# TDLdefA-QUN/Noise-Resilience-in-Discrete-Time-Crystal-Realizations-on-Quantum-Computers

Measured on AMD Instinct MI355X. Metric: Floquet-periods×instances/sec at L=20; RZZ-kernel HBM GB/s vs peak, higher is better.
Workload: dtype f64

## Files before the change

noise-resilience-in-discrete-time-crystal-realizations-on-quantum-computers_amd/csrc/dtc_lightcone.hip:

```cpp
#include <cstdlib>
#include <type_traits>

#include "dtc_device.h"
#include "dtc_kernels.h"

#ifndef DTC_LCW3_WPS
#if defined(DTC_LCW3_ADD) || defined(DTC_LCW3_MERGE)
#define DTC_LCW3_WPS 3
#else
#define DTC_LCW3_WPS 4
#endif
#endif
#ifndef DTC_LCW2_WPS
#define DTC_LCW2_WPS 4
#endif

namespace dtc {

static constexpr int kLcTilesPerGroup = 2;

template <int KIND, int TPB, bool SPLIT = false>
__device__ __forceinline__ void lc_body(const PassArgs& A) {
  static_assert(KIND == kKindRX || KIND == kKindRY, "light-cone pass: factored kicks");
  __shared__ double2 s_tile[SPLIT ? 1 : kTile];
  __shared__ double s_half[SPLIT ? kHalfSlots : 1];
  __shared__ double2 s_cone[kLcTab4];
  __shared__ double s_red[kThreads / 64][2];
  const int t = threadIdx.x;
  const int c = A.c, s = A.s;
  const int64_t n_tiles = (int64_t)1 << (A.L_eff - kTileBits);
  const int og = A.octet_bits;
  const int64_t b = og ? (((int64_t)blockIdx.y << 3) | (blockIdx.x & 7)) : (int64_t)blockIdx.y;
  const int64_t tile0 = (og ? (int64_t)(blockIdx.x >> 3) : (int64_t)blockIdx.x) * TPB;
  if (og && b >= A.batch) return;
  const int inst = (int)((A.batch_start + b) / A.n_traj);
  const RecScalar R(A.recs + b * kRecPerState);
  const int64_t mid_mask = ((int64_t)1 << A.tile_bits_mid) - 1;
  TileMap M;
  M.c = c;
  M.s = s;
  M.cmask = (1 << c) - 1;
  auto tbase_of = [&](int64_t tile) {
    return ((tile & mid_mask) << c) | ((tile >> A.tile_bits_mid) << (s + kTileBits - c));
  };
  M.tbase = tbase_of(tile0);
  constexpr int kConePerThread = (kLcTab4 + kThreads - 1) / kThreads;
  double2 cv[kConePerThread];
  const double2* ct = A.lc_diag + (int64_t)inst * kLcTab;
#pragma unroll
  for (int j = 0; j < kConePerThread; ++j) {
    const int i = t + j * kThreads;
    if (i < kLcTab4) cv[j] = ct[i];
  }
  const int64_t vofs = octet_spread(M.rel(ybase<2>(t)), og) << 4;
  const char* src = (const char*)(A.src + state_base(b, A.state_len, og));
  auto load_tile = [&](double2 (&dst)[kRegs], int64_t tb) {
#pragma unroll
    for (int r = 0; r < kRegs; ++r) {
      const char* a = src + (octet_spread(tb | M.rel(r << 8), og) << 4) + vofs;
      const d2v w = __builtin_nontemporal_load((const d2v*)a);
      dst[r] = make_double2(w.x, w.y);
    }
  };
  double2 v[kRegs];
  load_tile(v, M.tbase);
  __builtin_amdgcn_s_waitcnt(0x4F70);
  const double cs = A.diag_conj ? -1.0 : 1.0;
#pragma unroll
  for (int j = 0; j < kConePerThread; ++j) {
    const int i = t + j * kThreads;
    if (i < kLcTab4) s_cone[i] = make_double2(cv[j].x, cs * cv[j].y);
  }
  const double g2 = R.d(0, kLcG2);
  const long long packed = R.bits(kLcPacked);
  const int nl = A.lc_layers;
  const int jp = A.probe;

  auto kick = [&](double2 (&v)[kRegs], auto n_tag, auto l_tag) {
    constexpr int N = decltype(n_tag)::value;
    constexpr int l = decltype(l_tag)::value;
    constexpr int k0 = kLcSites * l + 4 * (N - 1);
    const int m = (int)((A.lc_mask >> k0) & 0xFull);
    if (m & 1) layer_f<KIND, 0, 0>(v, R.d(0, k0));
    if (m & 2) layer_f<KIND, 0, 1>(v, R.d(0, k0 + 1));
    if (m & 4) layer_f<KIND, 0, 2>(v, R.d(0, k0 + 2));
    if (m & 8) layer_f<KIND, 0, 3>(v, R.d(0, k0 + 3));
  };
  auto diag = [&](double2 (&v)[kRegs], auto lay_tag, int l) {
    constexpr int LAY = decltype(lay_tag)::value;
    const int rad = nl - 1 - l;
    const int lo = max(0, jp - rad), hi = min(A.L_real - 1, jp + rad);
    const int msk = (1 << (hi - lo + 1)) - 1;
    const int g0 = s + 4 * LAY - c;
    const int64_t m = (int64_t)((packed >> (8 * l)) & 0xFF) << s;
    const int base = (int)(((M.at(ybase<LAY>(t)) ^ m) >> lo) & msk);
    const double2* tab = s_cone + lc_tab_off(rad);
#pragma unroll
    for (int r = 0; r < kRegs; ++r) {
      const int off = (g0 >= lo ? (r << (g0 - lo)) : (r >> (lo - g0))) & msk;
      const int i = base ^ off;
      v[r] = cmul(v[r], tab[rad == 4 ? lc_pos4(i) : i]);
    }
  };
  using L1 = std::integral_constant<int, 1>;
  using L2 = std::integral_constant<int, 2>;
  auto lc_xch_impl = [&](double2 (&v)[kRegs], auto from_tag, auto to_tag) {
    constexpr int F = decltype(from_tag)::value, T = decltype(to_tag)::value;
    if constexpr (SPLIT) exchange_split<F, T>(v, s_half, t);
    else exchange<F, T>(v, s_tile, t);
  };
  auto process = [&](double2 (&v)[kRegs], int64_t tile) {
    M.tbase = tbase_of(tile);
    kick(v, L2{}, std::integral_constant<int, 0>{});
    lc_xch_impl(v, std::integral_constant<int, 2>{}, std::integral_constant<int, 1>{});
    kick(v, L1{}, std::integral_constant<int, 0>{});
    if (nl > 1) {
      diag(v, L1{}, 0);
      kick(v, L1{}, std::integral_constant<int, 1>{});
      lc_xch_impl(v, std::integral_constant<int, 1>{}, std::integral_constant<int, 2>{});
      kick(v, L2{}, std::integral_constant<int, 1>{});
    }
    if (nl > 2) {
      diag(v, L2{}, 1);
      kick(v, L2{}, std::integral_constant<int, 2>{});
      lc_xch_impl(v, std::integral_constant<int, 2>{}, std::integral_constant<int, 1>{});
      kick(v, L1{}, std::integral_constant<int, 2>{});
    }
    if (nl > 3) {
      diag(v, L1{}, 2);
      kick(v, L1{}, std::integral_constant<int, 3>{});
      lc_xch_impl(v, std::integral_constant<int, 1>{}, std::integral_constant<int, 2>{});
      kick(v, L2{}, std::integral_constant<int, 3>{});
    }
    if (nl > 4) {
      diag(v, L2{}, 3);
      kick(v, L2{}, std::integral_constant<int, 4>{});
      lc_xch_impl(v, std::integral_constant<int, 2>{}, std::integral_constant<int, 1>{});
      kick(v, L1{}, std::integral_constant<int, 4>{});
    }
    const int lay = (nl & 1) ? 1 : 2;
    double ptot = 0.0, pz = 0.0;
    {
      const int64_t x0 = lay == 1 ? M.at(ybase<1>(t)) : M.at(ybase<2>(t));
      const int tb = jp < c ? jp : ((jp >= s && jp < s + kTileBits - c) ? c + jp - s : -1);
      const int jr = tb - 4 * lay;
#pragma unroll
      for (int r = 0; r < kRegs; ++r) {
        const double p2 = fma(v[r].x, v[r].x, v[r].y * v[r].y);
        ptot += p2;
        pz += (jr >= 0 && jr < 4 && ((r >> jr) & 1)) ? -p2 : p2;
      }
      if (!(jr >= 0 && jr < 4)) pz = ((x0 >> jp) & 1) ? -ptot : ptot;
      if ((packed >> (32 + jp - s)) & 1) pz = -pz;
    }
    const int wave = t >> 6, lane = t & 63;
    const double tot = wave_sum(ptot) * g2;
    const double z = wave_sum(pz) * g2;
    if (lane == 0) {
      s_red[wave][0] = tot;
      s_red[wave][1] = z;
    }
    __syncthreads();
    if (t < 2) {
      double acc = 0.0;
// ... 358 lines not shown
#pragma unroll
    for (int p = 4; p < 12; ++p) xl |= (uint32_t)((t >> (p - 4)) & 1) << gpos(lay_site(kL0, p));
    const int64_t vofs = octet_spread((int64_t)xl, og) << 4;
    const char* src = (const char*)(A.src + state_base(b, A.state_len, og));
    const int64_t sp0 = octet_spread((int64_t)tbase, og) << 4;
    int64_t spq[4];
#pragma unroll
    for (int q = 0; q < 4; ++q) spq[q] = octet_spread((int64_t)1 << gpos(lay_site(kL0, q)), og) << 4;
#pragma unroll
    for (int r = 0; r < kRegs; ++r) {
      int64_t o = sp0;
#pragma unroll
      for (int q = 0; q < 4; ++q)
        if ((r >> q) & 1) o += spq[q];
      const d2v w = *(const d2v*)(src + o + vofs);
      v[r] = make_double2(w.x, w.y);
    }
  }
  const double2* ct = A.lc_diag + (int64_t)inst * kLcTab;
  auto tab_of = [](int e) {
    return e >= tab_off(kT1) ? kT1 : e >= tab_off(kT2) ? kT2 : e >= tab_off(kT3) ? kT3
         : e >= tab_off(kT4b) ? kT4b : e >= tab_off(kT4a) ? kT4a : e >= tab_off(kT5b) ? kT5b : kT5a;
  };
  auto tab_start = [](int k) {
    return k == kT5a ? tab_off(kT5a) : k == kT5b ? tab_off(kT5b) : k == kT4a ? tab_off(kT4a)
         : k == kT4b ? tab_off(kT4b) : k == kT3 ? tab_off(kT3) : k == kT2 ? tab_off(kT2) : tab_off(kT1);
  };
  auto src_of = [](int k) {
    return k == kT5a ? tab_src(kT5a) : k == kT5b ? tab_src(kT5b) : k == kT4a ? tab_src(kT4a)
         : k == kT4b ? tab_src(kT4b) : k == kT3 ? tab_src(kT3) : k == kT2 ? tab_src(kT2) : tab_src(kT1);
  };
  const int e1 = t + kThreads;
  const int k0 = tab_of(t), k1 = tab_of(e1);
  const int i0 = t - tab_start(k0), i1 = e1 - tab_start(k1);
  const double2 tv0 = ct[src_of(k0) + (k0 == kT5a ? lc_pos5a(i0) : i0)];
  double2 tv1 = make_double2(0.0, 0.0);
  if (e1 < kTabEntries) tv1 = ct[src_of(k1) + i1];
  kick(C0{}, C0{}, LCW2_SITE(m2));
  kick(C1{}, C0{}, LCW2_SITE(m1));
  kick(C2{}, C0{}, LCW2_SITE(z0));
  kick(C3{}, C0{}, LCW2_SITE(p1));
  {
    const double cs = A.diag_conj ? -1.0 : 1.0;
    const uint64_t m0 = (uint64_t)R.bits(kLcwMask + 0), m1 = (uint64_t)R.bits(kLcwMask + 1);
    const uint64_t m2 = (uint64_t)R.bits(kLcwMask + 2), m3 = (uint64_t)R.bits(kLcwMask + 3);
    const uint64_t m4 = (uint64_t)R.bits(kLcwMask + 4);
    auto stage = [&](int k, int i, double2 tv) {
      const int l = tab_layer(k);
      const uint64_t m = l == 0 ? m0 : l == 1 ? m1 : l == 2 ? m2 : l == 3 ? m3 : m4;
      const int lo = k == kT5a ? -5 : k == kT4a ? -4 : k == kT3 ? -3 : k == kT2 ? -2 : k == kT1 ? -1 : 0;
      const int nb = k == kT3 ? 7 : (k == kT5a || k == kT5b) ? 6 : k == kT1 ? 3 : 5;
      const int x = i ^ (int)((m >> (j + lo)) & ((1u << nb) - 1u));
      const int pos = k == kT5a ? (((x & 7) << 3) | (x >> 3))
                    : k == kT3 ? (((x & 15) << 2) | ((x >> 4) & 3) | (x & 64)) : x;
      s_tab[tab_start(k) + pos] = make_double2(tv.x, cs * tv.y);
    };
    stage(k0, i0, tv0);
    if (e1 < kTabEntries) stage(k1, i1, tv1);
  }

  xch(std::integral_constant<int, kL0>{}, std::integral_constant<int, kL1>{});
  kick(C0{}, C0{}, LCW2_SITE(m5));
  kick(C1{}, C0{}, LCW2_SITE(m4));
  kick(C2{}, C0{}, LCW2_SITE(m3));
  {
    int ba = tab_base<kL1, kT5a>(t, bit_p5), bb = tab_base<kL1, kT5b>(t, bit_p5);
    asm volatile("" : "+v"(ba), "+v"(bb));
    const double2* ta = s_tab + tab_off(kT5a) + ba;
    const double2* tb = s_tab + tab_off(kT5b) + bb;
#pragma unroll
    for (int r = 0; r < 8; ++r) {
      const double2 f = ta[tab_reg<kL1, kT5a>(r)];
      v[r] = cmul(v[r], f);
      v[r + 8] = cmul(v[r + 8], f);
    }
    const double2 f0 = tb[0], f1 = tb[tab_reg<kL1, kT5b>(8)];
#pragma unroll
    for (int r = 0; r < 8; ++r) {
      v[r] = cmul(v[r], f0);
      v[r + 8] = cmul(v[r + 8], f1);
    }
  }
  kick(C1{}, C1{}, LCW2_SITE(m4));
  kick(C2{}, C1{}, LCW2_SITE(m3));
  kick(C3{}, C1{}, LCW2_SITE(p4));
  xch(std::integral_constant<int, kL1>{}, std::integral_constant<int, kL2s>{});
  kick(C0{}, C1{}, LCW2_SITE(m2));
  kick(C1{}, C1{}, LCW2_SITE(m1));
  kick(C2{}, C1{}, LCW2_SITE(z0));
  kick(C3{}, C1{}, LCW2_SITE(p1));
  swap_reg_lane<0, 16>(v);
  swap_reg_lane<1, 32>(v);
  kick(C0{}, C1{}, LCW2_SITE(p2));
  kick(C1{}, C1{}, LCW2_SITE(p3));
  {
    int ba = tab_base<kL2e, kT4a>(t, bit_p5), bb = tab_base<kL2e, kT4b>(t, bit_p5);
    asm volatile("" : "+v"(ba), "+v"(bb));
    const double2* ta = s_tab + tab_off(kT4a) + ba;
    const double2* tb = s_tab + tab_off(kT4b) + bb;
    const double2 a0 = ta[0], a1 = ta[tab_reg<kL2e, kT4a>(4)];
#pragma unroll
    for (int r = 0; r < kRegs; ++r) v[r] = cmul(v[r], cmul((r & 4) ? a1 : a0, tb[tab_reg<kL2e, kT4b>(r)]));
  }
  kick(C0{}, C2{}, LCW2_SITE(p2));
  kick(C1{}, C2{}, LCW2_SITE(p3));
  kick(C2{}, C2{}, LCW2_SITE(z0));
  kick(C3{}, C2{}, LCW2_SITE(p1));
  xch(std::integral_constant<int, kL2e>{}, std::integral_constant<int, kL3s>{});
  kick(C0{}, C2{}, LCW2_SITE(m3));
  kick(C1{}, C2{}, LCW2_SITE(m2));
  kick(C2{}, C2{}, LCW2_SITE(m1));
  diag1(std::integral_constant<int, kL3s>{}, std::integral_constant<int, kT3>{});
  kick(C1{}, C3{}, LCW2_SITE(m2));
  kick(C2{}, C3{}, LCW2_SITE(m1));
  kick(C3{}, C3{}, LCW2_SITE(z0));
  swap_reg_lane<0, 32>(v);
  kick(C0{}, C3{}, LCW2_SITE(p1));
  swap_reg_lane<1, 16>(v);
  kick(C1{}, C3{}, LCW2_SITE(p2));
  diag1(std::integral_constant<int, kL3e>{}, std::integral_constant<int, kT2>{});
  kick(C2{}, C4{}, LCW2_SITE(m1));
  kick(C3{}, C4{}, LCW2_SITE(z0));
  kick(C0{}, C4{}, LCW2_SITE(p1));
  diag1(std::integral_constant<int, kL3e>{}, std::integral_constant<int, kT1>{});
  kick(C3{}, C5{}, LCW2_SITE(z0));
#undef LCW2_SITE
  double ptot = 0.0, pz = 0.0;
#pragma unroll
  for (int r = 0; r < kRegs; ++r) {
    const double p2v = fma(v[r].x, v[r].x, v[r].y * v[r].y);
    ptot += p2v;
    pz += ((r >> 3) & 1) ? -p2v : p2v;
  }
  if ((R.bits(kLcwMask + kLcwLayers - 1) >> j) & 1) pz = -pz;
  const double g2 = R.d(0, kLcwG2);
  const int wave = t >> 6, lane = t & 63;
  const double tot = wave_sum(ptot) * g2;
  const double z = wave_sum(pz) * g2;
  if (lane == 0) {
    s_red[wave][0] = tot;
    s_red[wave][1] = z;
  }
  __syncthreads();
  if (t < 2) {
    double acc = 0.0;
    for (int k = 0; k < kThreads / 64; ++k) acc += s_red[k][t];
    A.partial[(b * n_tiles + tile) * A.n_obs + t] = acc;
  }
}

namespace lcw3 {
enum : int { m5 = 0, m4, m3, m2, m1, z0, p1, p2, p3, p4, p5, p6, kNSite };
__host__ __device__ constexpr int off_of(int s) { return s - z0; }
#ifdef DTC_LCW3_ADD
__host__ __device__ constexpr int pos_of_site(int s) {
  return s == m4 ? 0 : s == m3 ? 1 : s == m2 ? 2 : s == m1 ? 3 : s == z0 ? 4 : s == p3 ? 5
       : s == p1 ? 6 : s == p5 ? 7 : s == p6 ? 8 : s == p2 ? 9 : s == m5 ? 10 : 11;
}
__host__ __device__ constexpr int cv(int s) {
  return (1 << pos_of_site(s)) + (pos_of_site(s) >= 5 ? 1 << (pos_of_site(s) - 5) : 0) +
         (pos_of_site(s) >= 10 ? 1 << (pos_of_site(s) - 10) : 0);
}
static constexpr int kSlots = 4226;
#define LCW3_SLOT(a, b) ((a) + (b))
#else
__host__ __device__ constexpr int cv(int s) {
  return s == m4 ? 1 : s == m3 ? 2 : s == m2 ? 4 : s == m1 ? 8 : s == z0 ? 16 | 1
       : s == p3 ? 32 | 2 : s == p4 ? 64 | 1 : s == p1 ? 128 | 2 : s == p5 ? 256 | 14
       : s == p6 ? 512 | 8 : s == p2 ? 1024 | 16 : 2048;
}
static constexpr int kSlots = kTile;
#define LCW3_SLOT(a, b) ((a) ^ (b))
#endif
enum : int { kX1 = 0, kX1e, kX1f, kX2, kX2s, kX3, kX3e, kX4, kX4e };
__host__ __device__ constexpr int lay_site(int li, int pos) {
  constexpr int tab[9][12] = {
      {p3, p4, p5, p6, m4, m3, m2, m1, p2, m5, z0, p1},
      {p3, p4, p5, p2, m4, m3, m2, m1, p6, m5, z0, p1},
      {m5, p4, p5, p2, m4, m3, m2, m1, p6, p3, z0, p1},
      {m4, m3, m2, m1, p3, p4, p5, p6, z0, p1, m5, p2},
      {z0, p1, m2, m1, p3, p4, p5, p6, m4, m3, m5, p2},
      {p2, p3, p4, m3, p1, m2, m1, z0, m4, m5, p5, p6},
      {p2, p3, m4, m3, p1, m2, m1, z0, p4, m5, p5, p6},
      {m2, m1, z0, p1, m4, m3, p5, p6, p2, m5, p3, p4},
      {p2, m1, z0, p1, m4, m3, p5, p6, m2, m5, p3, p4}};
  return tab[li][pos];
}
__host__ __device__ constexpr int reg_slot(int li, int r) {
  return LCW3_SLOT(LCW3_SLOT(LCW3_SLOT((r & 1) ? cv(lay_site(li, 0)) : 0,
                                       (r & 2) ? cv(lay_site(li, 1)) : 0),
                             (r & 4) ? cv(lay_site(li, 2)) : 0),
                   (r & 8) ? cv(lay_site(li, 3)) : 0);
}
template <int LI>
__device__ __forceinline__ int slot_base(int t) {
  int b = 0;
#pragma unroll
  for (int p = 4; p < 12; ++p) b = LCW3_SLOT(b, ((t >> (p - 4)) & 1) * cv(lay_site(LI, p)));
  return b;
}
enum : int { kT6a = 0, kT6b, kT5a, kT5b, kT4a, kT4b, kT3a, kT3b, kT2, kT1, kT4, kT3, kNTab };
__host__ __device__ constexpr int tab_off(int k) {
  return k == kT6a ? 0 : k == kT6b ? 64 : k == kT5a ? 192 : k == kT5b ? 256 : k == kT4a ? 320
       : k == kT4b ? 352 : k == kT3a ? 384 : k == kT3b ? 400 : k == kT2 ? 416 : k == kT1 ? 448
       : k == kT4 ? 456 : 968;
}
static constexpr int kTabStaged = 456;
#ifdef DTC_LCW3_MERGE
static constexpr int kTabEntries = 1096;
#else
static constexpr int kTabEntries = 456;
#endif
__host__ __device__ constexpr int tab_bits(int k) {
  return k == kT6a ? 6 : k == kT6b ? 7 : (k == kT5a || k == kT5b) ? 6 : (k == kT4a || k == kT4b) ? 5
       : (k == kT3a || k == kT3b) ? 4 : k == kT2 ? 5 : k == kT1 ? 3 : k == kT4 ? 9 : 7;
}
__host__ __device__ constexpr int tab_lo(int k) {
  return k == kT6a ? -5 : k == kT5a ? -5 : (k == kT4a || k == kT4) ? -4 : (k == kT3a || k == kT3) ? -3
       : k == kT2 ? -2 : k == kT1 ? -1 : 0;
}
__host__ __device__ constexpr int tab_layer(int k) {
  return (k == kT6a || k == kT6b) ? 0 : (k == kT5a || k == kT5b) ? 1 : (k == kT4a || k == kT4b) ? 2
       : (k == kT3a || k == kT3b) ? 3 : k == kT2 ? 4 : 5;
}
__host__ __device__ constexpr int tab_src(int k) {
  return k == kT6a ? kLcTab6a : k == kT6b ? kLcTab6b : k == kT5a ? kLcTab5a : k == kT5b ? kLcTab5b
       : k == kT4a ? kLcTab4a : k == kT4b ? kLcTab4b : k == kT3a ? kLcTab3a : k == kT3b ? kLcTab3b
       : lc_tab_off(k == kT2 ? 2 : 1);
}
__host__ __device__ constexpr int tab_wt(int k, int s) {
  const int d = off_of(s) - tab_lo(k);
  return (d < 0 || d >= tab_bits(k)) ? 0 : 1 << d;
}
template <int LI, int K>
__device__ __forceinline__ int tab_reg(int r) {
  return ((r & 1) ? tab_wt(K, lay_site(LI, 0)) : 0) + ((r & 2) ? tab_wt(K, lay_site(LI, 1)) : 0) +
         ((r & 4) ? tab_wt(K, lay_site(LI, 2)) : 0) + ((r & 8) ? tab_wt(K, lay_site(LI, 3)) : 0);
}
template <int LI, int K>
__device__ __forceinline__ int tab_base(int t) {
  int b = 0;
#pragma unroll
  for (int p = 4; p < 12; ++p) b += ((t >> (p - 4)) & 1) * tab_wt(K, lay_site(LI, p));
  return b;
}
}

template <int KIND>
__global__ __launch_bounds__(kThreads, DTC_LCW3_WPS) void dtc_lcw3_final(PassArgs A) {
  static_assert(KIND == kKindRX || KIND == kKindRY, "light-cone pass: factored kicks");
  using namespace lcw3;
  __shared__ double s_x[kSlots];
  __shared__ double2 s_tab[kTabEntries];
  __shared__ double s_red[kThreads / 64][2];
  const int t = threadIdx.x;
  const int64_t n_tiles = (int64_t)1 << (A.L_eff - kTileBits);
  const int og = A.octet_bits;
  const int64_t b = og ? (((int64_t)blockIdx.y << 3) | (blockIdx.x & 7)) : (int64_t)blockIdx.y;
  const int64_t tile = og ? (int64_t)(blockIdx.x >> 3) : (int64_t)blockIdx.x;
  if (og && b >= A.batch) return;
  const int inst = (int)((A.batch_start + b) / A.n_traj);
  const int j = A.probe;
  const RecScalar R(A.recs + b * kRecPerState);
  auto gpos = [&](int s) { return j + off_of(s); };
  const uint32_t tbase = ((uint32_t)tile & ((1u << (j - 5)) - 1u)) |
                         (((uint32_t)tile >> (j - 5)) << (j + 7));
  const int b6 = (int)((tbase >> (j - 6)) & 1u);
  double2 v[kRegs];
  auto xch = [&](auto from_tag, auto to_tag) {
    constexpr int F = decltype(from_tag)::value, T = decltype(to_tag)::value;
    int bf = slot_base<F>(t), bt = slot_base<T>(t);
    asm volatile("" : "+v"(bf), "+v"(bt));
#pragma unroll
    for (int r = 0; r < kRegs; ++r) s_x[LCW3_SLOT(bf, reg_slot(F, r))] = v[r].x;
    __syncthreads();
#pragma unroll
    for (int r = 0; r < kRegs; ++r) v[r].x = s_x[LCW3_SLOT(bt, reg_slot(T, r))];
    __syncthreads();
#pragma unroll
    for (int r = 0; r < kRegs; ++r) s_x[LCW3_SLOT(bf, reg_slot(F, r))] = v[r].y;
    __syncthreads();
#pragma unroll
    for (int r = 0; r < kRegs; ++r) v[r].y = s_x[LCW3_SLOT(bt, reg_slot(T, r))];
  };
  auto kick = [&](auto q_tag, auto l_tag, auto s_tag) {
    constexpr int Q = decltype(q_tag)::value, l = decltype(l_tag)::value, S = decltype(s_tag)::value;
    layer_f<KIND, 0, Q>(v, R.d(0, 12 * l + S));
  };
  auto diag2 = [&](auto lay_tag, auto ka_tag, auto kb_tag) {
    constexpr int LI = decltype(lay_tag)::value, KA = decltype(ka_tag)::value,
                  KB = decltype(kb_tag)::value;
    int ba = tab_base<LI, KA>(t), bb = tab_base<LI, KB>(t);
    asm volatile("" : "+v"(ba), "+v"(bb));
    const double2* ta = s_tab + tab_off(KA) + ba;
    const double2* tb = s_tab + tab_off(KB) + bb;
#pragma unroll
    for (int r = 0; r < kRegs; ++r)
      v[r] = cmul(v[r], cmul(ta[tab_reg<LI, KA>(r)], tb[tab_reg<LI, KB>(r)]));
  };
  auto diag1 = [&](auto lay_tag, auto k_tag) {
    constexpr int LI = decltype(lay_tag)::value, K = decltype(k_tag)::value;
    int base = tab_base<LI, K>(t);
    asm volatile("" : "+v"(base));
    const double2* tab = s_tab + tab_off(K) + base;
#pragma unroll
    for (int r = 0; r < kRegs; ++r) v[r] = cmul(v[r], tab[tab_reg<LI, K>(r)]);
  };
  using C0 = std::integral_constant<int, 0>;
  using C1 = std::integral_constant<int, 1>;
  using C2 = std::integral_constant<int, 2>;
  using C3 = std::integral_constant<int, 3>;
  using C4 = std::integral_constant<int, 4>;
  using C5 = std::integral_constant<int, 5>;
  using C6 = std::integral_constant<int, 6>;
#define LCW3_S(s) std::integral_constant<int, s>{}
#define LCW3_L(x) std::integral_constant<int, x>{}
  {
    uint32_t xl = 0;
#pragma unroll
    for (int p = 4; p < 12; ++p) xl |= (uint32_t)((t >> (p - 4)) & 1) << gpos(lay_site(kX1, p));
    const int64_t vofs = octet_spread((int64_t)xl, og) << 4;
    const char* src = (const char*)(A.src + state_base(b, A.state_len, og));
    const int64_t sp0 = octet_spread((int64_t)tbase, og) << 4;
    int64_t spq[4];
#pragma unroll
    for (int q = 0; q < 4; ++q) spq[q] = octet_spread((int64_t)1 << gpos(lay_site(kX1, q)), og) << 4;
    const bool vofs32 = vofs < ((int64_t)1 << 32);
#pragma unroll
    for (int r = 0; r < kRegs; ++r) {
      int64_t o = sp0;
#pragma unroll
      for (int q = 0; q < 4; ++q)
        if ((r >> q) & 1) o += spq[q];
      const d2v w = vofs32 ? *(const d2v*)(src + o + (uint32_t)vofs) : *(const d2v*)(src + o + vofs);
      v[r] = make_double2(w.x, w.y);
    }
  }
  const double2* ct = A.lc_diag + (int64_t)inst * kLcTab;
  auto src_of = [&](auto k_tag, int i) {
    constexpr int K = decltype(k_tag)::value;
    return tab_src(K) + (K == kT6a ? ((i << 1) | b6) : K == kT5a ? lc_pos5a(i) : i);
  };
  auto dst_of = [&](auto k_tag, int i) {
    constexpr int K = decltype(k_tag)::value;
    const uint64_t m = (uint64_t)R.bits(kLcw3Mask + tab_layer(K));
    return tab_off(K) + (i ^ (int)((m >> (j + tab_lo(K))) & ((1u << tab_bits(K)) - 1u)));
  };
  using K6a = std::integral_constant<int, kT6a>;
  using K6b = std::integral_constant<int, kT6b>;
  using K5a = std::integral_constant<int, kT5a>;
  using K5b = std::integral_constant<int, kT5b>;
  using K4a = std::integral_constant<int, kT4a>;
  using K4b = std::integral_constant<int, kT4b>;
  using K3a = std::integral_constant<int, kT3a>;
  using K3b = std::integral_constant<int, kT3b>;
  using K2 = std::integral_constant<int, kT2>;
  using K1 = std::integral_constant<int, kT1>;
  static_assert(tab_off(kT6b) == 64 && tab_off(kT5a) == 192 && tab_off(kT5b) == 256 &&
                    tab_off(kT4a) == 320 && tab_off(kT4b) == 352 && tab_off(kT3a) == 384 &&
                    tab_off(kT3b) == 400 && tab_off(kT2) == 416 && tab_off(kT1) == 448 &&
                    kTabStaged == 456 && kThreads == 256,
                "the per-wave table split below");
  const int wv = __builtin_amdgcn_readfirstlane(t >> 6), ln = t & 63;
  int s0, d0, s1 = -1, d1 = 0;
  if (wv == 0) {
    s0 = src_of(K6a{}, ln); d0 = dst_of(K6a{}, ln);
    s1 = src_of(K5b{}, ln); d1 = dst_of(K5b{}, ln);
  } else if (wv == 1) {
    s0 = src_of(K6b{}, ln); d0 = dst_of(K6b{}, ln);
    const bool a = ln < 32;
    s1 = a ? src_of(K4a{}, ln) : src_of(K4b{}, ln - 32);
    d1 = a ? dst_of(K4a{}, ln) : dst_of(K4b{}, ln - 32);
  } else if (wv == 2) {
    s0 = src_of(K6b{}, 64 + ln); d0 = dst_of(K6b{}, 64 + ln);
    s1 = ln < 16 ? src_of(K3a{}, ln) : ln < 32 ? src_of(K3b{}, ln - 16) : src_of(K2{}, ln - 32);
    d1 = ln < 16 ? dst_of(K3a{}, ln) : ln < 32 ? dst_of(K3b{}, ln - 16) : dst_of(K2{}, ln - 32);
  } else {
    s0 = src_of(K5a{}, ln); d0 = dst_of(K5a{}, ln);
    if (ln < 8) {
      s1 = src_of(K1{}, ln);
      d1 = dst_of(K1{}, ln);
    }
  }
  const double2 tv0 = ct[s0];
  double2 tv1 = make_double2(0.0, 0.0);
  if (s1 >= 0) tv1 = ct[s1];
  kick(C0{}, C0{}, LCW3_S(p3));
  kick(C1{}, C0{}, LCW3_S(p4));
  kick(C2{}, C0{}, LCW3_S(p5));
  kick(C3{}, C0{}, LCW3_S(p6));
  swap_reg_lane<3, 16>(v);
  if ((A.lc_mask >> p2) & 1ull) kick(C3{}, C0{}, LCW3_S(p2));
  {
    const double cs = A.diag_conj ? -1.0 : 1.0;
    s_tab[d0] = make_double2(tv0.x, cs * tv0.y);
    if (s1 >= 0) s_tab[d1] = make_double2(tv1.x, cs * tv1.y);
  }
  __syncthreads();
  diag2(LCW3_L(kX1e), LCW3_L(kT6a), LCW3_L(kT6b));
  kick(C0{}, C1{}, LCW3_S(p3));
  kick(C1{}, C1{}, LCW3_S(p4));
  kick(C2{}, C1{}, LCW3_S(p5));
  kick(C3{}, C1{}, LCW3_S(p2));
  swap_reg_lane<0, 32>(v);
  kick(C0{}, C1{}, LCW3_S(m5));
#ifdef DTC_LCW3_MERGE
#pragma unroll
  for (int e = 0; e < 2; ++e) {
    const int y = t + e * kThreads;
    s_tab[tab_off(kT4) + y] = cmul(s_tab[tab_off(kT4a) + (y & 31)], s_tab[tab_off(kT4b) + (y >> 4)]);
  }
  if (t < 128) s_tab[tab_off(kT3) + t] = cmul(s_tab[tab_off(kT3a) + (t & 15)], s_tab[tab_off(kT3b) + (t >> 3)]);
#endif
  xch(LCW3_L(kX1f), LCW3_L(kX2));
  kick(C0{}, C1{}, LCW3_S(m4));
  kick(C1{}, C1{}, LCW3_S(m3));
  kick(C2{}, C1{}, LCW3_S(m2));
  kick(C3{}, C1{}, LCW3_S(m1));
  swap_reg_lane<0, 16>(v);
  swap_reg_lane<1, 32>(v);
  kick(C0{}, C1{}, LCW3_S(z0));
  kick(C1{}, C1{}, LCW3_S(p1));
  diag2(LCW3_L(kX2s), LCW3_L(kT5a), LCW3_L(kT5b));
  kick(C0{}, C2{}, LCW3_S(z0));
  kick(C1{}, C2{}, LCW3_S(p1));
  kick(C2{}, C2{}, LCW3_S(m2));
  kick(C3{}, C2{}, LCW3_S(m1));
  xch(LCW3_L(kX2s), LCW3_L(kX3));
  kick(C0{}, C2{}, LCW3_S(p2));
  kick(C1{}, C2{}, LCW3_S(p3));
  kick(C2{}, C2{}, LCW3_S(p4));
  kick(C3{}, C2{}, LCW3_S(m3));
  swap_reg_lane<2, 16>(v);
  kick(C2{}, C2{}, LCW3_S(m4));
#ifdef DTC_LCW3_MERGE
  diag1(LCW3_L(kX3e), LCW3_L(kT4));
#else
  diag2(LCW3_L(kX3e), LCW3_L(kT4a), LCW3_L(kT4b));
#endif
  kick(C0{}, C3{}, LCW3_S(p2));
  kick(C1{}, C3{}, LCW3_S(p3));
  kick(C3{}, C3{}, LCW3_S(m3));
  xch(LCW3_L(kX3e), LCW3_L(kX4));
  kick(C0{}, C3{}, LCW3_S(m2));
  kick(C1{}, C3{}, LCW3_S(m1));
  kick(C2{}, C3{}, LCW3_S(z0));
  kick(C3{}, C3{}, LCW3_S(p1));
#ifdef DTC_LCW3_MERGE
  diag1(LCW3_L(kX4), LCW3_L(kT3));
#else
  diag2(LCW3_L(kX4), LCW3_L(kT3a), LCW3_L(kT3b));
#endif
  kick(C0{}, C4{}, LCW3_S(m2));
  kick(C1{}, C4{}, LCW3_S(m1));
  kick(C2{}, C4{}, LCW3_S(z0));
  kick(C3{}, C4{}, LCW3_S(p1));
  swap_reg_lane<0, 16>(v);
  kick(C0{}, C4{}, LCW3_S(p2));
  diag1(LCW3_L(kX4e), LCW3_L(kT2));
  kick(C1{}, C5{}, LCW3_S(m1));
  kick(C2{}, C5{}, LCW3_S(z0));
  kick(C3{}, C5{}, LCW3_S(p1));
  diag1(LCW3_L(kX4e), LCW3_L(kT1));
  kick(C2{}, C6{}, LCW3_S(z0));
#undef LCW3_S
#undef LCW3_L
  double ptot = 0.0, pz = 0.0;
#pragma unroll
  for (int r = 0; r < kRegs; ++r) {
    const double p2v = fma(v[r].x, v[r].x, v[r].y * v[r].y);
    ptot += p2v;
    pz += ((r >> 2) & 1) ? -p2v : p2v;
  }
  if ((R.bits(kLcw3Mask + kLcw3Layers - 1) >> j) & 1) pz = -pz;
  const double g2 = R.d(0, kLcw3G2);
  const int wave = t >> 6, lane = t & 63;
  const double tot = wave_sum(ptot) * g2;
  const double z = wave_sum(pz) * g2;
  if (lane == 0) {
    s_red[wave][0] = tot;
    s_red[wave][1] = z;
  }
  __syncthreads();
  int t2 = t;
  asm volatile("" : "+v"(t2));
  if (t2 < 2) {
    double acc = 0.0;
    for (int k = 0; k < kThreads / 64; ++k) acc += s_red[k][t2];
    A.partial[(b * n_tiles + tile) * A.n_obs + t2] = acc;
  }
}

hipError_t launch_lightcone(const PassArgs& a, dim3 grid, int kind, hipStream_t stream,
                            int* variant) {
  int vdummy = 0;
  if (!variant) variant = &vdummy;
  const int n_tiles = 1 << (a.L_eff - kTileBits);
  if (a.lc_wide == 2) {
    const int j = a.probe;
    if (a.meas != kMeasProbe || !a.no_store || a.lc_layers != kLcw3Layers || a.n_obs < 2 ||
        !a.lc_diag || j < 6 || j + 6 > a.L_real - 1 || a.L_eff > 32 ||
        (kind != kKindRX && kind != kKindRY))
      return hipErrorInvalidValue;
    for (int k = 0; k < kTileBits; ++k)
      if (a.lc_gb[k] != j - 5 + k) return hipErrorInvalidValue;
    *variant = kLcVariantWide3;
    hipLaunchKernelGGL((kind == kKindRX ? dtc_lcw3_final<kKindRX> : dtc_lcw3_final<kKindRY>), grid,
                       dim3(kThreads), 0, stream, a);
    return hipGetLastError();
  }
  if (a.lc_wide) {
    if (a.meas != kMeasProbe || !a.no_store || a.lc_layers != kLcwLayers || a.n_obs < 2 ||
        !a.lc_diag || a.lc_gb[0] != 0 || a.lc_gb[1] != 1 || a.lc_gb[6] != a.probe ||
        (kind != kKindRX && kind != kKindRY))
      return hipErrorInvalidValue;
    uint64_t seen = 0;
    for (int k = 0; k < kTileBits; ++k) {
      if (a.lc_gb[k] < 0 || a.lc_gb[k] >= a.L_eff || ((seen >> a.lc_gb[k]) & 1)) return hipErrorInvalidValue;
      seen |= 1ull << a.lc_gb[k];
    }
    const int j = a.probe;
    const int8_t canon[kTileBits] = {0, 1, (int8_t)(j - 5), (int8_t)(j + 4), (int8_t)(j - 2),
                                     (int8_t)(j - 1), (int8_t)j, (int8_t)(j + 1), (int8_t)(j + 2),
                                     (int8_t)(j + 3), (int8_t)(j - 4), (int8_t)(j - 3)};
    bool lcw2 = a.lc_mask == kLcwMaskJ2 && j >= 7 && j + 5 <= a.L_real - 1 && a.lc_tpb >= 0;
    for (int k = 0; k < kTileBits && lcw2; ++k) lcw2 = a.lc_gb[k] == canon[k];
    *variant = lcw2 ? kLcVariantWide2 : kLcVariantWide;
    if (lcw2)
      hipLaunchKernelGGL((kind == kKindRX ? dtc_lcw2_final<kKindRX> : dtc_lcw2_final<kKindRY>), grid,
                         dim3(kThreads), 0, stream, a);
    else if (a.lc_mask == kLcwMaskJ2)
      hipLaunchKernelGGL((kind == kKindRX ? dtc_lcw_final<kKindRX, kLcwMaskJ2>
                                          : dtc_lcw_final<kKindRY, kLcwMaskJ2>),
                         grid, dim3(kThreads), 0, stream, a);
    else
      hipLaunchKernelGGL((kind == kKindRX ? dtc_lcw_final<kKindRX> : dtc_lcw_final<kKindRY>), grid,
                         dim3(kThreads), 0, stream, a);
    return hipGetLastError();
  }
  {
    *variant = kLcVariant8;
    if (a.c != 4 || a.act != 0xFF0 || a.meas != kMeasProbe || !a.no_store || a.lc_layers < 1 ||
        a.lc_layers > kLcLayers || a.n_obs < 2 || !a.lc_diag)
      return hipErrorInvalidValue;
    int tpb = a.lc_tpb > 0 ? a.lc_tpb : kLcTilesPerGroup;
    if (a.lc_split) {
      if (kind != kKindRX && kind != kKindRY) return hipErrorInvalidValue;
      hipLaunchKernelGGL((kind == kKindRX ? dtc_lc_final_split<kKindRX> : dtc_lc_final_split<kKindRY>),
                         grid, dim3(kThreads), 0, stream, a);
      return hipGetLastError();
    }
    while (tpb > 1 && n_tiles % tpb) tpb >>= 1;
    if (tpb != 1 && tpb != 2 && tpb != 4) tpb = 1;
    grid.x = (a.octet_bits ? 8 : 1) * n_tiles / tpb;
    if (kind != kKindRX && kind != kKindRY) return hipErrorInvalidValue;
    const bool rx = kind == kKindRX;
    if (tpb == 4)
      hipLaunchKernelGGL((rx ? dtc_lc_final<kKindRX, 4> : dtc_lc_final<kKindRY, 4>), grid, dim3(kThreads), 0, stream, a);
    else if (tpb == 2)
      hipLaunchKernelGGL((rx ? dtc_lc_final<kKindRX, 2> : dtc_lc_final<kKindRY, 2>), grid, dim3(kThreads), 0, stream, a);
    else
      hipLaunchKernelGGL((rx ? dtc_lc_final<kKindRX, 1> : dtc_lc_final<kKindRY, 1>), grid, dim3(kThreads), 0, stream, a);
    return hipGetLastError();
  }
}

}
```

Before: 257,000.

## Use per-exchange swizzled LDS slot maps and bitfield address math in lcw3 kernel

Replaces the single shared-memory swizzle used for all three register re-layouts with a separate XOR-based slot map per exchange. Compile-time GF(2) rank checks assert each map is injective and conflict-free for 16-lane writes and 32-lane reads. Per-thread slot, table and load base offsets are now built with masked shifts over lane and wave bits instead of per-bit loops, and the 32-bit offset fast path is chosen from the maximum offset. The experimental ADD and MERGE variants are removed. The aim is to cut LDS bank conflicts and integer address arithmetic, at the cost of more complex constexpr machinery.

```diff
diff --git a/noise-resilience-in-discrete-time-crystal-realizations-on-quantum-computers_amd/csrc/dtc_lightcone.hip b/noise-resilience-in-discrete-time-crystal-realizations-on-quantum-computers_amd/csrc/dtc_lightcone.hip
--- a/noise-resilience-in-discrete-time-crystal-realizations-on-quantum-computers_amd/csrc/dtc_lightcone.hip
+++ b/noise-resilience-in-discrete-time-crystal-realizations-on-quantum-computers_amd/csrc/dtc_lightcone.hip
@@ -1,15 +1,12 @@
 #include <cstdlib>
 #include <type_traits>
+#include <utility>
 
 #include "dtc_device.h"
 #include "dtc_kernels.h"
 
 #ifndef DTC_LCW3_WPS
-#if defined(DTC_LCW3_ADD) || defined(DTC_LCW3_MERGE)
-#define DTC_LCW3_WPS 3
-#else
 #define DTC_LCW3_WPS 4
-#endif
 #endif
 #ifndef DTC_LCW2_WPS
 #define DTC_LCW2_WPS 4
@@ -674,27 +671,7 @@
 namespace lcw3 {
 enum : int { m5 = 0, m4, m3, m2, m1, z0, p1, p2, p3, p4, p5, p6, kNSite };
 __host__ __device__ constexpr int off_of(int s) { return s - z0; }
-#ifdef DTC_LCW3_ADD
-__host__ __device__ constexpr int pos_of_site(int s) {
-  return s == m4 ? 0 : s == m3 ? 1 : s == m2 ? 2 : s == m1 ? 3 : s == z0 ? 4 : s == p3 ? 5
-       : s == p1 ? 6 : s == p5 ? 7 : s == p6 ? 8 : s == p2 ? 9 : s == m5 ? 10 : 11;
-}
-__host__ __device__ constexpr int cv(int s) {
-  return (1 << pos_of_site(s)) + (pos_of_site(s) >= 5 ? 1 << (pos_of_site(s) - 5) : 0) +
-         (pos_of_site(s) >= 10 ? 1 << (pos_of_site(s) - 10) : 0);
-}
-static constexpr int kSlots = 4226;
-#define LCW3_SLOT(a, b) ((a) + (b))
-#else
-__host__ __device__ constexpr int cv(int s) {
-  return s == m4 ? 1 : s == m3 ? 2 : s == m2 ? 4 : s == m1 ? 8 : s == z0 ? 16 | 1
-       : s == p3 ? 32 | 2 : s == p4 ? 64 | 1 : s == p1 ? 128 | 2 : s == p5 ? 256 | 14
-       : s == p6 ? 512 | 8 : s == p2 ? 1024 | 16 : 2048;
-}
-static constexpr int kSlots = kTile;
-#define LCW3_SLOT(a, b) ((a) ^ (b))
-#endif
-enum : int { kX1 = 0, kX1e, kX1f, kX2, kX2s, kX3, kX3e, kX4, kX4e };
+enum : int { kX1 = 0, kX1e, kX1f, kX2, kX2s, kX3, kX3e, kX4, kX4e, kNLay };
 __host__ __device__ constexpr int lay_site(int li, int pos) {
   constexpr int tab[9][12] = {
       {p3, p4, p5, p6, m4, m3, m2, m1, p2, m5, z0, p1},
@@ -708,37 +685,147 @@
       {p2, m1, z0, p1, m4, m3, p5, p6, m2, m5, p3, p4}};
   return tab[li][pos];
 }
-__host__ __device__ constexpr int reg_slot(int li, int r) {
-  return LCW3_SLOT(LCW3_SLOT(LCW3_SLOT((r & 1) ? cv(lay_site(li, 0)) : 0,
-                                       (r & 2) ? cv(lay_site(li, 1)) : 0),
-                             (r & 4) ? cv(lay_site(li, 2)) : 0),
-                   (r & 8) ? cv(lay_site(li, 3)) : 0);
-}
-template <int LI>
-__device__ __forceinline__ int slot_base(int t) {
-  int b = 0;
-#pragma unroll
-  for (int p = 4; p < 12; ++p) b = LCW3_SLOT(b, ((t >> (p - 4)) & 1) * cv(lay_site(LI, p)));
-  return b;
-}
-enum : int { kT6a = 0, kT6b, kT5a, kT5b, kT4a, kT4b, kT3a, kT3b, kT2, kT1, kT4, kT3, kNTab };
+enum : int { kE1 = 0, kE2, kE3, kNXch };
+__host__ __device__ constexpr int xch_from(int e) { return e == kE1 ? kX1f : e == kE2 ? kX2s : kX3e; }
+__host__ __device__ constexpr int xch_to(int e) { return e == kE1 ? kX2 : e == kE2 ? kX3 : kX4; }
+__host__ __device__ constexpr int cv(int e, int s) {
+  constexpr int tab[kNXch][kNSite] = {
+      {2048, 1,       2,      4,      8,  512 | 2, 1024,   64,   32 | 1, 16,  128 | 4, 256 | 8},
+      {1024, 512 | 4, 128,    64 | 2, 16, 256 | 8, 32 | 1, 2048, 1,      2,   4,       8},
+      {1024, 32 | 1,  64 | 2, 2,      4,  8,       1,      16,   2048,   512, 128 | 4, 256 | 8}};
+  return tab[e][s];
+}
+static constexpr int kSlots = kTile;
+__host__ __device__ constexpr bool site_private(int e, int s) {
+  int others = 0;
+  for (int q = 0; q < kNSite; ++q)
+    if (q != s) others |= cv(e, q);
+  return (cv(e, s) & others) == 0;
+}
+__host__ __device__ constexpr int reg_xor(int e, int li, int r) {
+  int x = 0;
+  for (int q = 0; q < 4; ++q)
+    if (((r >> q) & 1) && !site_private(e, lay_site(li, q))) x ^= cv(e, lay_site(li, q));
+  return x;
+}
+__host__ __device__ constexpr int reg_slot(int e, int li, int r) {
+  int x = 0;
+  for (int q = 0; q < 4; ++q)
+    if ((r >> q) & 1) x ^= cv(e, lay_site(li, q));
+  return x;
+}
+__host__ __device__ constexpr int reg_add(int e, int li, int r) {
+  int a = 0;
+  for (int q = 0; q < 4; ++q)
+    if (((r >> q) & 1) && site_private(e, lay_site(li, q))) a += cv(e, lay_site(li, q));
+  return a;
+}
+__host__ __device__ constexpr int gf2_rank(int e, int li, int p0, int n, int mask) {
+  int v[12] = {};
+  for (int i = 0; i < n; ++i) v[i] = cv(e, lay_site(li, p0 + i)) & mask;
+  int rk = 0;
+  for (int bit = 0; bit < 12 && rk < n; ++bit) {
+    int piv = -1;
+    for (int i = rk; i < n; ++i)
+      if ((v[i] >> bit) & 1) {
+        piv = i;
+        break;
+      }
+    if (piv < 0) continue;
+    const int tmp = v[piv];
+    v[piv] = v[rk];
+    v[rk] = tmp;
+    for (int i = 0; i < n; ++i)
+      if (i != rk && ((v[i] >> bit) & 1)) v[i] ^= v[rk];
+    ++rk;
+  }
+  return rk;
+}
+__host__ __device__ constexpr bool lay_is_permutation(int li) {
+  int seen = 0;
+  for (int p = 0; p < 12; ++p) seen |= 1 << lay_site(li, p);
+  return seen == (1 << kNSite) - 1;
+}
+__host__ __device__ constexpr bool all_layouts_permutations() {
+  for (int li = 0; li < kNLay; ++li)
+    if (!lay_is_permutation(li)) return false;
+  return true;
+}
+__host__ __device__ constexpr bool xch_injective(int e) {
+  int all = 0;
+  for (int s = 0; s < kNSite; ++s) all |= cv(e, s);
+  return all < kSlots && gf2_rank(e, xch_from(e), 0, 12, kSlots - 1) == 12 &&
+         gf2_rank(e, xch_to(e), 0, 12, kSlots - 1) == 12;
+}
+__host__ __device__ constexpr bool xch_writes_conflict_free(int e) {
+  return gf2_rank(e, xch_from(e), 4, 4, 15) == 4;
+}
+__host__ __device__ constexpr bool xch_reads_conflict_free(int e) {
+  return gf2_rank(e, xch_to(e), 4, 5, 31) == 5;
+}
+static_assert(all_layouts_permutations(), "every layout places each of the twelve sites once");
+static_assert(xch_injective(kE1) && xch_injective(kE2) && xch_injective(kE3),
+              "re-layout slot maps: 4096 distinct slots");
+static_assert(xch_writes_conflict_free(kE1) && xch_writes_conflict_free(kE2) &&
+                  xch_writes_conflict_free(kE3),
+              "re-layout writes: a 16-lane group covers 16 banks");
+static_assert(xch_reads_conflict_free(kE1) && xch_reads_conflict_free(kE2) &&
+                  xch_reads_conflict_free(kE3),
+              "re-layout reads: a 32-lane group covers 32 banks");
+template <class M>
+__host__ __device__ constexpr int lin_mask(int d) {
+  int m = 0;
+  for (int k = 0; k < M::kBits; ++k) {
+    const int o = k + d;
+    if (o >= 0 && o < 16 && ((M::vec(k) >> o) & 1)) m |= 1 << k;
+  }
+  return m;
+}
+template <class M, int D>
+__device__ __forceinline__ int lin_shift(int x) {
+  constexpr int m = lin_mask<M>(D);
+  if constexpr (m == 0)
+    return 0;
+  else if constexpr (D >= 0)
+    return (x & m) << D;
+  else
+    return (x & m) >> -D;
+}
+template <class M, int... I>
+__device__ __forceinline__ int lin_apply(int x, std::integer_sequence<int, I...>) {
+  return (0 ^ ... ^ lin_shift<M, I - 15>(x));
+}
+template <class M>
+__device__ __forceinline__ int lin_map(int x) {
+  return lin_apply<M>(x, std::make_integer_sequence<int, 31>{});
+}
+template <int E, int LI, int P0, int N>
+struct SlotVec {
+  static constexpr int kBits = N;
+  __host__ __device__ static constexpr int vec(int k) { return cv(E, lay_site(LI, P0 + k)); }
+};
+template <int E, int LI>
+__device__ __forceinline__ int slot_base(int ln, int wv) {
+  return lin_map<SlotVec<E, LI, 4, 6>>(ln) ^ lin_map<SlotVec<E, LI, 10, 2>>(wv);
+}
+template <int P0, int N>
+struct LoadVec {
+  static constexpr int kBits = N;
+  __host__ __device__ static constexpr int vec(int k) { return 1 << (off_of(lay_site(kX1, P0 + k)) + 5); }
+};
+enum : int { kT6a = 0, kT6b, kT5a, kT5b, kT4a, kT4b, kT3a, kT3b, kT2, kT1, kNTab };
 __host__ __device__ constexpr int tab_off(int k) {
   return k == kT6a ? 0 : k == kT6b ? 64 : k == kT5a ? 192 : k == kT5b ? 256 : k == kT4a ? 320
-       : k == kT4b ? 352 : k == kT3a ? 384 : k == kT3b ? 400 : k == kT2 ? 416 : k == kT1 ? 448
-       : k == kT4 ? 456 : 968;
+       : k == kT4b ? 352 : k == kT3a ? 384 : k == kT3b ? 400 : k == kT2 ? 416 : 448;
 }
 static constexpr int kTabStaged = 456;
-#ifdef DTC_LCW3_MERGE
-static constexpr int kTabEntries = 1096;
-#else
 static constexpr int kTabEntries = 456;
-#endif
 __host__ __device__ constexpr int tab_bits(int k) {
   return k == kT6a ? 6 : k == kT6b ? 7 : (k == kT5a || k == kT5b) ? 6 : (k == kT4a || k == kT4b) ? 5
-       : (k == kT3a || k == kT3b) ? 4 : k == kT2 ? 5 : k == kT1 ? 3 : k == kT4 ? 9 : 7;
+       : (k == kT3a || k == kT3b) ? 4 : k == kT2 ? 5 : 3;
 }
 __host__ __device__ constexpr int tab_lo(int k) {
-  return k == kT6a ? -5 : k == kT5a ? -5 : (k == kT4a || k == kT4) ? -4 : (k == kT3a || k == kT3) ? -3
+  return k == kT6a ? -5 : k == kT5a ? -5 : k == kT4a ? -4 : k == kT3a ? -3
        : k == kT2 ? -2 : k == kT1 ? -1 : 0;
 }
 __host__ __device__ constexpr int tab_layer(int k) {
@@ -759,12 +846,14 @@
   return ((r & 1) ? tab_wt(K, lay_site(LI, 0)) : 0) + ((r & 2) ? tab_wt(K, lay_site(LI, 1)) : 0) +
          ((r & 4) ? tab_wt(K, lay_site(LI, 2)) : 0) + ((r & 8) ? tab_wt(K, lay_site(LI, 3)) : 0);
 }
+template <int LI, int K, int P0, int N>
+struct TabVec {
+  static constexpr int kBits = N;
+  __host__ __device__ static constexpr int vec(int k) { return tab_wt(K, lay_site(LI, P0 + k)); }
+};
 template <int LI, int K>
-__device__ __forceinline__ int tab_base(int t) {
-  int b = 0;
-#pragma unroll
-  for (int p = 4; p < 12; ++p) b += ((t >> (p - 4)) & 1) * tab_wt(K, lay_site(LI, p));
-  return b;
+__device__ __forceinline__ int tab_base(int ln, int wv) {
+  return lin_map<TabVec<LI, K, 4, 6>>(ln) + lin_map<TabVec<LI, K, 10, 2>>(wv);
 }
 }
 
@@ -788,22 +877,23 @@
   const uint32_t tbase = ((uint32_t)tile & ((1u << (j - 5)) - 1u)) |
                          (((uint32_t)tile >> (j - 5)) << (j + 7));
   const int b6 = (int)((tbase >> (j - 6)) & 1u);
+  const int wv = __builtin_amdgcn_readfirstlane(t >> 6), ln = t & 63;
   double2 v[kRegs];
-  auto xch = [&](auto from_tag, auto to_tag) {
-    constexpr int F = decltype(from_tag)::value, T = decltype(to_tag)::value;
-    int bf = slot_base<F>(t), bt = slot_base<T>(t);
+  auto xch = [&](auto e_tag) {
+    constexpr int E = decltype(e_tag)::value, F = xch_from(E), T = xch_to(E);
+    int bf = slot_base<E, F>(ln, wv), bt = slot_base<E, T>(ln, wv);
     asm volatile("" : "+v"(bf), "+v"(bt));
 #pragma unroll
-    for (int r = 0; r < kRegs; ++r) s_x[LCW3_SLOT(bf, reg_slot(F, r))] = v[r].x;
+    for (int r = 0; r < kRegs; ++r) s_x[(bf ^ reg_xor(E, F, r)) + reg_add(E, F, r)] = v[r].x;
     __syncthreads();
 #pragma unroll
-    for (int r = 0; r < kRegs; ++r) v[r].x = s_x[LCW3_SLOT(bt, reg_slot(T, r))];
+    for (int r = 0; r < kRegs; ++r) v[r].x = s_x[bt ^ reg_slot(E, T, r)];
     __syncthreads();
 #pragma unroll
-    for (int r = 0; r < kRegs; ++r) s_x[LCW3_SLOT(bf, reg_slot(F, r))] = v[r].y;
+    for (int r = 0; r < kRegs; ++r) s_x[(bf ^ reg_xor(E, F, r)) + reg_add(E, F, r)] = v[r].y;
     __syncthreads();
 #pragma unroll
-    for (int r = 0; r < kRegs; ++r) v[r].y = s_x[LCW3_SLOT(bt, reg_slot(T, r))];
+    for (int r = 0; r < kRegs; ++r) v[r].y = s_x[bt ^ reg_slot(E, T, r)];
   };
   auto kick = [&](auto q_tag, auto l_tag, auto s_tag) {
     constexpr int Q = decltype(q_tag)::value, l = decltype(l_tag)::value, S = decltype(s_tag)::value;
@@ -812,7 +902,7 @@
   auto diag2 = [&](auto lay_tag, auto ka_tag, auto kb_tag) {
     constexpr int LI = decltype(lay_tag)::value, KA = decltype(ka_tag)::value,
                   KB = decltype(kb_tag)::value;
-    int ba = tab_base<LI, KA>(t), bb = tab_base<LI, KB>(t);
+    int ba = tab_base<LI, KA>(ln, wv), bb = tab_base<LI, KB>(ln, wv);
     asm volatile("" : "+v"(ba), "+v"(bb));
     const double2* ta = s_tab + tab_off(KA) + ba;
     const double2* tb = s_tab + tab_off(KB) + bb;
@@ -822,7 +912,7 @@
   };
   auto diag1 = [&](auto lay_tag, auto k_tag) {
     constexpr int LI = decltype(lay_tag)::value, K = decltype(k_tag)::value;
-    int base = tab_base<LI, K>(t);
+    int base = tab_base<LI, K>(ln, wv);
     asm volatile("" : "+v"(base));
     const double2* tab = s_tab + tab_off(K) + base;
 #pragma unroll
@@ -838,25 +928,31 @@
 #define LCW3_S(s) std::integral_constant<int, s>{}
 #define LCW3_L(x) std::integral_constant<int, x>{}
   {
-    uint32_t xl = 0;
-#pragma unroll
-    for (int p = 4; p < 12; ++p) xl |= (uint32_t)((t >> (p - 4)) & 1) << gpos(lay_site(kX1, p));
+    const uint32_t xl = (uint32_t)lin_map<LoadVec<4, 6>>(ln) << (j - 5);
+    const uint32_t xw = (uint32_t)lin_map<LoadVec<10, 2>>(wv) << (j - 5);
     const int64_t vofs = octet_spread((int64_t)xl, og) << 4;
     const char* src = (const char*)(A.src + state_base(b, A.state_len, og));
-    const int64_t sp0 = octet_spread((int64_t)tbase, og) << 4;
+    const int64_t sp0 = octet_spread((int64_t)(tbase | xw), og) << 4;
     int64_t spq[4];
 #pragma unroll
     for (int q = 0; q < 4; ++q) spq[q] = octet_spread((int64_t)1 << gpos(lay_site(kX1, q)), og) << 4;
-    const bool vofs32 = vofs < ((int64_t)1 << 32);
-#pragma unroll
-    for (int r = 0; r < kRegs; ++r) {
-      int64_t o = sp0;
-#pragma unroll
-      for (int q = 0; q < 4; ++q)
-        if ((r >> q) & 1) o += spq[q];
-      const d2v w = vofs32 ? *(const d2v*)(src + o + (uint32_t)vofs) : *(const d2v*)(src + o + vofs);
-      v[r] = make_double2(w.x, w.y);
-    }
+    const int64_t vmax =
+        octet_spread((int64_t)((uint32_t)lin_map<LoadVec<4, 6>>(63) << (j - 5)), og) << 4;
+    auto load_tile = [&](auto lane_ofs) {
+#pragma unroll
+      for (int r = 0; r < kRegs; ++r) {
+        int64_t o = sp0;
+#pragma unroll
+        for (int q = 0; q < 4; ++q)
+          if ((r >> q) & 1) o += spq[q];
+        const d2v w = *(const d2v*)(src + o + lane_ofs);
+        v[r] = make_double2(w.x, w.y);
+      }
+    };
+    if (vmax < ((int64_t)1 << 32))
+      load_tile((uint32_t)vofs);
+    else
+      load_tile(vofs);
   }
   const double2* ct = A.lc_diag + (int64_t)inst * kLcTab;
   auto src_of = [&](auto k_tag, int i) {
@@ -883,7 +979,6 @@
                     tab_off(kT3b) == 400 && tab_off(kT2) == 416 && tab_off(kT1) == 448 &&
                     kTabStaged == 456 && kThreads == 256,
                 "the per-wave table split below");
-  const int wv = __builtin_amdgcn_readfirstlane(t >> 6), ln = t & 63;
   int s0, d0, s1 = -1, d1 = 0;
   if (wv == 0) {
     s0 = src_of(K6a{}, ln); d0 = dst_of(K6a{}, ln);
@@ -926,15 +1021,7 @@
   kick(C3{}, C1{}, LCW3_S(p2));
   swap_reg_lane<0, 32>(v);
   kick(C0{}, C1{}, LCW3_S(m5));
-#ifdef DTC_LCW3_MERGE
-#pragma unroll
-  for (int e = 0; e < 2; ++e) {
-    const int y = t + e * kThreads;
-    s_tab[tab_off(kT4) + y] = cmul(s_tab[tab_off(kT4a) + (y & 31)], s_tab[tab_off(kT4b) + (y >> 4)]);
-  }
-  if (t < 128) s_tab[tab_off(kT3) + t] = cmul(s_tab[tab_off(kT3a) + (t & 15)], s_tab[tab_off(kT3b) + (t >> 3)]);
-#endif
-  xch(LCW3_L(kX1f), LCW3_L(kX2));
+  xch(LCW3_L(kE1));
   kick(C0{}, C1{}, LCW3_S(m4));
   kick(C1{}, C1{}, LCW3_S(m3));
   kick(C2{}, C1{}, LCW3_S(m2));
@@ -948,31 +1035,23 @@
   kick(C1{}, C2{}, LCW3_S(p1));
   kick(C2{}, C2{}, LCW3_S(m2));
   kick(C3{}, C2{}, LCW3_S(m1));
-  xch(LCW3_L(kX2s), LCW3_L(kX3));
+  xch(LCW3_L(kE2));
   kick(C0{}, C2{}, LCW3_S(p2));
   kick(C1{}, C2{}, LCW3_S(p3));
   kick(C2{}, C2{}, LCW3_S(p4));
   kick(C3{}, C2{}, LCW3_S(m3));
   swap_reg_lane<2, 16>(v);
   kick(C2{}, C2{}, LCW3_S(m4));
-#ifdef DTC_LCW3_MERGE
-  diag1(LCW3_L(kX3e), LCW3_L(kT4));
-#else
   diag2(LCW3_L(kX3e), LCW3_L(kT4a), LCW3_L(kT4b));
-#endif
   kick(C0{}, C3{}, LCW3_S(p2));
   kick(C1{}, C3{}, LCW3_S(p3));
   kick(C3{}, C3{}, LCW3_S(m3));
-  xch(LCW3_L(kX3e), LCW3_L(kX4));
+  xch(LCW3_L(kE3));
   kick(C0{}, C3{}, LCW3_S(m2));
   kick(C1{}, C3{}, LCW3_S(m1));
   kick(C2{}, C3{}, LCW3_S(z0));
   kick(C3{}, C3{}, LCW3_S(p1));
-#ifdef DTC_LCW3_MERGE
-  diag1(LCW3_L(kX4), LCW3_L(kT3));
-#else
   diag2(LCW3_L(kX4), LCW3_L(kT3a), LCW3_L(kT3b));
-#endif
   kick(C0{}, C4{}, LCW3_S(m2));
   kick(C1{}, C4{}, LCW3_S(m1));
   kick(C2{}, C4{}, LCW3_S(z0));
```

New measurement: 257,100 (median of 2 runs). Within noise of the previous version (+0.0%).
